# turbocast/HTS-train-WORLD

Measured on AMD Instinct MI355X. Metric: WORLD analysis+synthesis frames/sec @16kHz, 5ms hop, higher is better.
Workload: dtype f64

## Files before the change

### hts-train-world_amd/csrc/stonemask.hip

```cpp
#include "batch.hpp"
#include "common.hpp"
#include "fastmath.hpp"
#include "fft.hpp"
#include "partition.hpp"

namespace wm {

constexpr double kFloorF0StoneMask = 40.0;

constexpr int kSmTwid = 8192;
__global__ __launch_bounds__(256) void sm_twiddle_kernel(cpx* __restrict__ tw) {
  const int k = blockIdx.x * 256 + threadIdx.x;
  if (k < kSmTwid) tw[k] = cis_neg2pi((double)k / (double)kSmTwid);
}

struct StoneMaskPred {
  const double* f0;
  double upper;
  __device__ bool operator()(int i) const {
    const double f = f0[i];
    return f == f && !(f <= kFloorF0StoneMask || f > upper);
  }
};

struct SmFrame {
  const double* xu;
  int xl, hw, L, fftn, raw0;
  bool regular;
  double pos, fs, inv_fs, inv_wlen;
  __device__ __forceinline__ int raw(int i) const {
    return regular ? raw0 + i : matlab_round((pos + (double)(-hw + i) / fs) * fs);
  }
};

__device__ __forceinline__ double sm_blackman(double c) {
  return fma(c, fma(0.16, c, 0.5), 0.34);
}

template <int NB>
__device__ __forceinline__ void sm_walk(const SmFrame& fr, const int (&bin)[NB], const cpx* __restrict__ twid,
                                        double (&pw)[NB], double (&num)[NB]) {
  auto bin_twiddle = [&](int b) -> cpx {
    if (fr.fftn <= kSmTwid) return twid[(bin[b] & (fr.fftn - 1)) * (kSmTwid / fr.fftn)];
    return cis_neg2pi((double)(bin[b] & (fr.fftn - 1)) / (double)fr.fftn);
  };
  double coef[NB];
#pragma unroll
  for (int b = 0; b < NB; ++b) coef[b] = 2.0 * bin_twiddle(b).x;
  double m1[NB], m2[NB], d1[NB], d2[NB];
#pragma unroll
  for (int b = 0; b < NB; ++b) m1[b] = m2[b] = d1[b] = d2[b] = 0.0;
  double c, sn, cd, sd;
  int r_cur = fr.raw(0);
  wm_sincospi(2.0 * ((r_cur - 1.0) * fr.inv_fs - fr.pos) * fr.inv_wlen, &sn, &c);
  wm_sincospi(2.0 * fr.inv_fs * fr.inv_wlen, &sd, &cd);
  double w_prev = 0.0, w_cur = sm_blackman(c);
  const int L = fr.L;
  for (int i0 = 0; i0 < L; i0 += 4) {
    int rv[5];
    rv[0] = r_cur;
#pragma unroll
    for (int q = 1; q < 5; ++q) rv[q] = fr.raw(imin(i0 + q, L - 1));
    double xv[4];
    if (fr.regular && rv[0] >= 1 && rv[0] + 2 < fr.xl) {
      load4_a8(fr.xu + (rv[0] - 1), xv);
    } else {
#pragma unroll
      for (int q = 0; q < 4; ++q) xv[q] = fr.xu[imax(0, imin(fr.xl - 1, rv[q] - 1))];
    }
#pragma unroll
    for (int q = 0; q < 4; ++q) {
      const int i = i0 + q;
      double cn;
      if (fr.regular) {
        cn = c * cd - sn * sd;
        sn = sn * cd + c * sd;
      } else {
        cn = cospi(2.0 * ((rv[q + 1] - 1.0) * fr.inv_fs - fr.pos) * fr.inv_wlen);
      }
      c = cn;
      const double w_next = i + 1 < L ? sm_blackman(c) : 0.0;
      const double x = i < L ? xv[q] : 0.0;
      const double am = x * w_cur;
      const double ad = x * (0.5 * (w_prev - w_next));
#pragma unroll
      for (int b = 0; b < NB; ++b) {
        const double tm = fma(coef[b], m1[b], am - m2[b]);
        m2[b] = m1[b];
        m1[b] = tm;
        const double td = fma(coef[b], d1[b], ad - d2[b]);
        d2[b] = d1[b];
        d1[b] = td;
      }
      w_prev = w_cur;
      w_cur = w_next;
    }
    r_cur = rv[4];
  }
#pragma unroll
  for (int b = 0; b < NB; ++b) {
    const cpx t = bin_twiddle(b);
    const double cwb = t.x, swb = -t.y;
    const double mr = m1[b] - cwb * m2[b], mi = swb * m2[b];
    const double dr = d1[b] - cwb * d2[b], di = swb * d2[b];
    num[b] = mr * di - mi * dr;
    pw[b] = mr * mr + mi * mi;
  }
}

template <int NB>
__device__ __forceinline__ double sm_fix(const double (&pw)[NB], const double (&num)[NB], const int (&bin)[NB],
                                         int fftn, int fs) {
  const double inv_fftn = 1.0 / fftn;
  const double fs_over_2pi = fs / 2.0 / kPi;
  double numer = 0.0, denom = 0.0;
#pragma unroll
  for (int h = 0; h < NB; ++h) {
    const double p = bin[h] <= fftn / 2 ? pw[h] : 0.0;
    const double inst = p == 0.0 ? 0.0 : (double)bin[h] * fs * inv_fftn + num[h] / p * fs_over_2pi;
    const double amp = sqrt(p);
    numer += amp * inst;
    denom += amp * (h + 1);
  }
  return numer / (denom + kSafe);
}

constexpr int kSmChunk = 256;
constexpr int kSmBins = 2048;

__global__ __launch_bounds__(256) void stonemask_kernel(
    const double* __restrict__ x, const int64_t* __restrict__ x_off, const int* __restrict__ x_len,
    const int* __restrict__ frame_utt, const double* __restrict__ tpos, const double* __restrict__ f0, int fs,
    const int* __restrict__ perm, const int* __restrict__ n_listed, const cpx* __restrict__ twid,
    double* __restrict__ out) {
  __shared__ int hist[kSmBins];
  __shared__ unsigned short order[kSmChunk];
  __shared__ int sh_w[4];
  const int tid = threadIdx.x, lane = tid & 63, wv = tid >> 6;
  const int n_run = *n_listed;
  const float hw_scale = 1.5f * (float)fs;
  for (int64_t c0 = (int64_t)blockIdx.x * kSmChunk; c0 < n_run; c0 += (int64_t)gridDim.x * kSmChunk) {
    for (int b = tid; b < kSmBins; b += 256) hist[b] = 0;
    __syncthreads();
    const bool mine = c0 + tid < n_run;
    int key = 0, rank = 0;
    if (mine) {
      const float fv = (float)f0[perm[c0 + tid]];
      key = kSmBins - 1 - imin(kSmBins - 1, (int)(hw_scale * __frcp_rn(fv) + 1.0f));
      rank = atomicAdd(&hist[key], 1);
    }
    __syncthreads();
    {
      int4 c4a = reinterpret_cast<int4*>(hist)[2 * tid], c4b = reinterpret_cast<int4*>(hist)[2 * tid + 1];
      const int minesum = c4a.x + c4a.y + c4a.z + c4a.w + c4b.x + c4b.y + c4b.z + c4b.w;
      const int incl = wave_scan_incl_i(minesum);
      if (lane == 63) sh_w[wv] = incl;
      __syncthreads();
      int base = incl - minesum;
      for (int q = 0; q < wv; ++q) base += sh_w[q];
      int4 oa, ob;
      oa.x = base; oa.y = oa.x + c4a.x; oa.z = oa.y + c4a.y; oa.w = oa.z + c4a.z;
      ob.x = oa.w + c4a.w; ob.y = ob.x + c4b.x; ob.z = ob.y + c4b.y; ob.w = ob.z + c4b.z;
      reinterpret_cast<int4*>(hist)[2 * tid] = oa;
      reinterpret_cast<int4*>(hist)[2 * tid + 1] = ob;
    }
    __syncthreads();
    if (mine) order[hist[key] + rank] = (unsigned short)tid;
    __syncthreads();
    const int n_here = (int)(n_run - c0 < kSmChunk ? n_run - c0 : kSmChunk);
    if (tid < n_here) {
      const int64_t frame = perm[c0 + order[tid]];
      const double f = f0[frame];
      const int u = frame_utt[frame];
      SmFrame fr;
      fr.xu = x + x_off[u];
      fr.xl = x_len[u];
      fr.pos = tpos[frame];
      fr.fs = fs;
      fr.inv_fs = 1.0 / fs;
      fr.hw = (int)(1.5 * fs / f + 1.0);
      fr.L = 2 * fr.hw + 1;
      fr.inv_wlen = fs / (2.0 * fr.hw + 1.0);
      fr.fftn = 1 << (2 + (31 - __clz(fr.L)));
      const double q = fr.pos * fs;
      fr.regular = fabs(q - floor(q) - 0.5) > 1e-6;
      fr.raw0 = matlab_round((fr.pos + (double)(-fr.hw) / fs) * fs);
      int bin2[2];
      double pw2[2], num2[2];
#pragma unroll
      for (int h = 0; h < 2; ++h) bin2[h] = matlab_round(f * fr.fftn / fs * (h + 1));
      sm_walk<2>(fr, bin2, twid, pw2, num2);
      const double tent = sm_fix<2>(pw2, num2, bin2, fr.fftn, fs);
      double mean = 0.0;
      if (!(tent <= 0.0 || tent > f * 2)) {
        int bin6[6];
        double pw6[6], num6[6];
#pragma unroll
        for (int h = 0; h < 6; ++h) bin6[h] = matlab_round(tent * fr.fftn / fs * (h + 1));
        sm_walk<6>(fr, bin6, twid, pw6, num6);
        mean = sm_fix<6>(pw6, num6, bin6, fr.fftn, fs);
      }
      if (fabs(mean - f) / f > 0.2) mean = f;
      out[frame] = mean;
    }
    __syncthreads();
  }
}

int launch_stonemask(Batch& b, const double* d_x, const double* d_t, const double* d_f0, double* d_out,
                     double f0_lower) {
  (void)f0_lower;
  Context& c = *b.ctx;
  const int fs = b.p.fs;
  const int64_t tf = b.total_f;
  if (tf <= 0) return WM_OK;
  const Table* twid = nullptr;
  int rc = c.table({kSmTwiddles, {}}, twid, [&](Table& t) {
    int r = wm_check(t.alloc(&t.d[0], sizeof(cpx) * (size_t)kSmTwid));
    if (r) return r;
    hipLaunchKernelGGL(sm_twiddle_kernel, dim3(kSmTwid / 256), dim3(256), 0, c.stream, (cpx*)t.d[0]);
    r = wm_check(hipGetLastError());
    return r ? r : wm_check(hipStreamSynchronize(c.stream));
  });
  if (rc) return rc;
  if (d_out == d_f0) {
    set_error("StoneMask: refined_f0 must not alias f0");
    return WM_ERR_BAD_ARG;
  }
  rc = wm_check(hipMemsetAsync(d_out, 0, sizeof(double) * (size_t)tf, c.stream));
  if (rc) return rc;
  TimedScope ts_(b.ctx, c.stream, "stonemask_kernel");
  launch_partition(c.stream, StoneMaskPred{d_f0, fs / 12.0}, (int)tf, b.d_part_cnt, b.d_perm, b.d_part_n);
  const int64_t chunks = (tf + kSmChunk - 1) / kSmChunk;
  const int64_t cap = (int64_t)c.num_cu * 64;
  hipLaunchKernelGGL(stonemask_kernel, dim3((unsigned)(chunks < cap ? chunks : cap)), dim3(256), 0, c.stream, d_x, b.d_x_off,
                     b.d_x_len, b.d_frame_utt, d_t, d_f0, fs, (const int*)b.d_perm, (const int*)b.d_part_n,
                     (const cpx*)twid->d[0], d_out);
  return wm_check(hipGetLastError());
}

}
```

Measured before the change: 21.49 million.

## Split each StoneMask Goertzel walk across four lanes and combine with DPP

Each frame's Goertzel recurrence over its window is split into four contiguous segments, each handled by a separate lane. Every partial result is phase-rotated by the twiddle for the samples that follow it, and the four partials are summed with DPP lane shuffles. This shortens the serial per-thread loop and spreads long windows over more lanes, so the stage has more parallel work. The cost is 64 frames per block chunk instead of 256, so the histogram, scan and sync setup runs four times as often per frame, plus extra twiddle work per segment. A launch-bounds occupancy hint of three blocks per multiprocessor is also added.

```diff
diff --git a/hts-train-world_amd/csrc/stonemask.hip b/hts-train-world_amd/csrc/stonemask.hip
--- a/hts-train-world_amd/csrc/stonemask.hip
+++ b/hts-train-world_amd/csrc/stonemask.hip
@@ -37,26 +37,43 @@
   return fma(c, fma(0.16, c, 0.5), 0.34);
 }
 
+constexpr int kSmParts = 4;
+
+__device__ __forceinline__ double sm_parts_sum(double v) {
+  static_assert(kSmParts == 2 || kSmParts == 4 || kSmParts == 8, "lanes that the DPP steps below add");
+  v += dpp_get<0xB1, 0xf, 0xf>(v);
+  if constexpr (kSmParts >= 4) v += dpp_get<0x4E, 0xf, 0xf>(v);
+  if constexpr (kSmParts >= 8) v += dpp_get<0x141, 0xf, 0xf>(v);
+  return v;
+}
+
 template <int NB>
-__device__ __forceinline__ void sm_walk(const SmFrame& fr, const int (&bin)[NB], const cpx* __restrict__ twid,
-                                        double (&pw)[NB], double (&num)[NB]) {
-  auto bin_twiddle = [&](int b) -> cpx {
-    if (fr.fftn <= kSmTwid) return twid[(bin[b] & (fr.fftn - 1)) * (kSmTwid / fr.fftn)];
-    return cis_neg2pi((double)(bin[b] & (fr.fftn - 1)) / (double)fr.fftn);
+__device__ __forceinline__ void sm_walk(const SmFrame& fr, int part, const int (&bin)[NB],
+                                        const cpx* __restrict__ twid, double (&pw)[NB], double (&num)[NB]) {
+  auto twiddle = [&](unsigned k) -> cpx {
+    k &= (unsigned)(fr.fftn - 1);
+    if (fr.fftn <= kSmTwid) return twid[k * (unsigned)(kSmTwid / fr.fftn)];
+    return cis_neg2pi((double)k / (double)fr.fftn);
   };
   double coef[NB];
 #pragma unroll
-  for (int b = 0; b < NB; ++b) coef[b] = 2.0 * bin_twiddle(b).x;
+  for (int b = 0; b < NB; ++b) coef[b] = 2.0 * twiddle((unsigned)bin[b]).x;
   double m1[NB], m2[NB], d1[NB], d2[NB];
 #pragma unroll
   for (int b = 0; b < NB; ++b) m1[b] = m2[b] = d1[b] = d2[b] = 0.0;
+  const int L = fr.L;
+  const int Lp = (L + 4 * kSmParts - 1) / (4 * kSmParts) * 4;
+  const int i_begin = part * Lp, i_end = imin(i_begin + Lp, L);
   double c, sn, cd, sd;
-  int r_cur = fr.raw(0);
+  int r_cur = fr.raw(imin(i_begin, L - 1));
   wm_sincospi(2.0 * ((r_cur - 1.0) * fr.inv_fs - fr.pos) * fr.inv_wlen, &sn, &c);
   wm_sincospi(2.0 * fr.inv_fs * fr.inv_wlen, &sd, &cd);
   double w_prev = 0.0, w_cur = sm_blackman(c);
-  const int L = fr.L;
-  for (int i0 = 0; i0 < L; i0 += 4) {
+  if (i_begin > 0 && i_begin < L)
+    w_prev = sm_blackman(fr.regular ? c * cd + sn * sd
+                                    : cospi(2.0 * ((fr.raw(i_begin - 1) - 1.0) * fr.inv_fs - fr.pos) * fr.inv_wlen));
+  int i0 = i_begin;
+  for (; i0 < i_end; i0 += 4) {
     int rv[5];
     rv[0] = r_cur;
 #pragma unroll
@@ -97,12 +114,20 @@
     }
     r_cur = rv[4];
   }
+  const unsigned behind = (unsigned)(kSmParts * Lp - i0);
 #pragma unroll
   for (int b = 0; b < NB; ++b) {
-    const cpx t = bin_twiddle(b);
+    const cpx t = twiddle((unsigned)bin[b]);
     const double cwb = t.x, swb = -t.y;
-    const double mr = m1[b] - cwb * m2[b], mi = swb * m2[b];
-    const double dr = d1[b] - cwb * d2[b], di = swb * d2[b];
+    double mr = m1[b] - cwb * m2[b], mi = swb * m2[b];
+    double dr = d1[b] - cwb * d2[b], di = swb * d2[b];
+    const cpx r = twiddle((unsigned)bin[b] * behind);
+    const double mr2 = mr * r.x + mi * r.y, mi2 = mi * r.x - mr * r.y;
+    const double dr2 = dr * r.x + di * r.y, di2 = di * r.x - dr * r.y;
+    mr = sm_parts_sum(mr2);
+    mi = sm_parts_sum(mi2);
+    dr = sm_parts_sum(dr2);
+    di = sm_parts_sum(di2);
     num[b] = mr * di - mi * dr;
     pw[b] = mr * mr + mi * mi;
   }
@@ -125,10 +150,10 @@
   return numer / (denom + kSafe);
 }
 
-constexpr int kSmChunk = 256;
+constexpr int kSmChunk = 256 / kSmParts;
 constexpr int kSmBins = 2048;
 
-__global__ __launch_bounds__(256) void stonemask_kernel(
+__global__ __launch_bounds__(256, 3) void stonemask_kernel(
     const double* __restrict__ x, const int64_t* __restrict__ x_off, const int* __restrict__ x_len,
     const int* __restrict__ frame_utt, const double* __restrict__ tpos, const double* __restrict__ f0, int fs,
     const int* __restrict__ perm, const int* __restrict__ n_listed, const cpx* __restrict__ twid,
@@ -142,7 +167,7 @@
   for (int64_t c0 = (int64_t)blockIdx.x * kSmChunk; c0 < n_run; c0 += (int64_t)gridDim.x * kSmChunk) {
     for (int b = tid; b < kSmBins; b += 256) hist[b] = 0;
     __syncthreads();
-    const bool mine = c0 + tid < n_run;
+    const bool mine = tid < kSmChunk && c0 + tid < n_run;
     int key = 0, rank = 0;
     if (mine) {
       const float fv = (float)f0[perm[c0 + tid]];
@@ -168,8 +193,9 @@
     if (mine) order[hist[key] + rank] = (unsigned short)tid;
     __syncthreads();
     const int n_here = (int)(n_run - c0 < kSmChunk ? n_run - c0 : kSmChunk);
-    if (tid < n_here) {
-      const int64_t frame = perm[c0 + order[tid]];
+    if (tid / kSmParts < n_here) {
+      const int part = tid % kSmParts;
+      const int64_t frame = perm[c0 + order[tid / kSmParts]];
       const double f = f0[frame];
       const int u = frame_utt[frame];
       SmFrame fr;
@@ -189,7 +215,7 @@
       double pw2[2], num2[2];
 #pragma unroll
       for (int h = 0; h < 2; ++h) bin2[h] = matlab_round(f * fr.fftn / fs * (h + 1));
-      sm_walk<2>(fr, bin2, twid, pw2, num2);
+      sm_walk<2>(fr, part, bin2, twid, pw2, num2);
       const double tent = sm_fix<2>(pw2, num2, bin2, fr.fftn, fs);
       double mean = 0.0;
       if (!(tent <= 0.0 || tent > f * 2)) {
@@ -197,11 +223,11 @@
         double pw6[6], num6[6];
 #pragma unroll
         for (int h = 0; h < 6; ++h) bin6[h] = matlab_round(tent * fr.fftn / fs * (h + 1));
-        sm_walk<6>(fr, bin6, twid, pw6, num6);
+        sm_walk<6>(fr, part, bin6, twid, pw6, num6);
         mean = sm_fix<6>(pw6, num6, bin6, fr.fftn, fs);
       }
       if (fabs(mean - f) / f > 0.2) mean = f;
-      out[frame] = mean;
+      if (part == 0) out[frame] = mean;
     }
     __syncthreads();
   }
@@ -231,7 +257,7 @@
   if (rc) return rc;
   TimedScope ts_(b.ctx, c.stream, "stonemask_kernel");
   launch_partition(c.stream, StoneMaskPred{d_f0, fs / 12.0}, (int)tf, b.d_part_cnt, b.d_perm, b.d_part_n);
-  const int64_t chunks = (tf + kSmChunk - 1) / kSmChunk;
+  const int64_t chunks = (tf + 255) / 256;
   const int64_t cap = (int64_t)c.num_cu * 64;
   hipLaunchKernelGGL(stonemask_kernel, dim3((unsigned)(chunks < cap ? chunks : cap)), dim3(256), 0, c.stream, d_x, b.d_x_off,
                      b.d_x_len, b.d_frame_utt, d_t, d_f0, fs, (const int*)b.d_perm, (const int*)b.d_part_n,
```

New measurement: 22.01 million, median of 6. About the same (+2.4%).
